# rensonnetg/microstructure_fingerprinting

Hardware: AMD Instinct MI355X
Metric: voxels/sec, 2-fascicle exhaustive NNLS, 782-atom x 200-measurement dictionary (higher is better)
Workload: dtype f64 (pairs ranked on split-f16 MFMA, short list re-evaluated in f64); 1 GPU; C2: 100000 voxels/GPU, 2 fascicles, 782 atoms x 200 measurements; voxels_per_gpu=100000, global_voxels=100000, atoms=782, measurements=200, ranks_in_group=1

## Files before the change

### microstructure_fingerprinting_amd/_lib.py

```python
import ctypes as C
import os

import numpy as np

_HERE = os.path.dirname(os.path.abspath(__file__))
LIB_PATH = os.path.join(_HERE, "libmfx.so")

MFX_OK, MFX_ERR_ARG, MFX_ERR_G_RANGE, MFX_ERR_NO_DEVICE, MFX_ERR_HIP, MFX_ERR_UNSUPPORTED, MFX_ERR_DIR_NORM = range(7)

_lib = None

EXPORTS = [
    "mfx_last_error", "mfx_device_count", "mfx_abi_version",
    "mfx_tables_create", "mfx_tables_destroy", "mfx_tables_num_atoms",
    "mfx_plan_create_multishell", "mfx_plan_create_explicit", "mfx_plan_destroy", "mfx_plan_status",
    "mfx_rotate", "mfx_rotate_dev", "mfx_rotate_cols", "mfx_rotate_cols_dev", "mfx_fit_batch", "mfx_fit_batch_rows", "mfx_fit_batch_volume", "mfx_volume_rows", "mfx_thread_release", "mfx_fit_batch_dev",
    "mfx_solve_exhaustive", "mfx_monte_carlo_average", "mfx_monte_carlo_average_dev", "mfx_cleanup_2fascicles", "mfx_cleanup_2fascicles_dev", "mfx_last_kernel_ms", "mfx_set_profiling", "mfx_debug_set_stamps", "mfx_debug_last_fallback_count", "mfx_debug_last_guard_count", "mfx_debug_last_counter", "mfx_debug_set_k2_screen", "mfx_debug_set_k2_wide", "mfx_debug_set_k2x_screen", "mfx_debug_set_k2_maxc", "mfx_debug_set_k2x_maxc", "mfx_debug_set_k2s_cap", "mfx_debug_set_k2s_images", "mfx_debug_set_k3_cap", "mfx_debug_set_force_generic", "mfx_debug_set_k3_screen",
]

MCF_EXPORTS = ["mfx_mcf_abi_version", "mfx_mcf_pgse", "mfx_mcf_dde"]

ROT2D_EXPORTS = ["mfx_rot2d_abi_version", "mfx_rot2d_create", "mfx_rot2d_destroy", "mfx_rot2d_rotate",
                 "mfx_rot2d_rotate_dev", "mfx_rot2d_rotate_cols", "mfx_rot2d_rotate_cols_dev"]

FIT2D_EXPORTS = ["mfx_fit2d_abi_version", "mfx_fit2d_max_atoms", "mfx_fit2d_batch_dev", "mfx_fit2d_batch",
                 "mfx_fit2d_debug_set_force_explicit"]

WFIT_EXPORTS = ["mfx_wfit_abi_version", "mfx_wfit_max_atoms", "mfx_wfit_batch_dev", "mfx_wfit_batch",
                "mfx_wfit_debug_set_force_explicit"]

PREDICT_EXPORTS = ["mfx_predict_abi_version", "mfx_predict_dev", "mfx_predict", "mfx_sos_noise_dev", "mfx_sos_noise"]

PROFILE_EXPORTS = ["mfx_profile_abi_version", "mfx_profile_cut", "mfx_profile_max_atoms", "mfx_profile_dev", "mfx_profile",
                   "mfx_pair_objectives_dev", "mfx_pair_objectives", "mfx_profile_debug_last_config"]

POST_EXPORTS = ["mfx_post_abi_version", "mfx_post_max_atoms", "mfx_post_dev", "mfx_post", "mfx_post_debug_last_config"]

WSOFT_EXPORTS = ["mfx_wsoft_abi_version", "mfx_wsoft_max_atoms", "mfx_wpost_dev", "mfx_wpost", "mfx_wprofile_dev", "mfx_wprofile",
                 "mfx_wpair_objectives_dev", "mfx_wpair_objectives"]

SOFT2D_EXPORTS = ["mfx_soft2d_abi_version", "mfx_soft2d_max_atoms", "mfx_post2d_dev", "mfx_post2d", "mfx_profile2d_dev",
# ... 80 lines not shown
    L.mfx_debug_last_guard_count.restype = C.c_int
    L.mfx_debug_last_counter.argtypes = [C.c_int]
    L.mfx_debug_last_counter.restype = C.c_int
    L.mfx_debug_set_k2x_maxc.argtypes = [C.c_int]
    L.mfx_debug_set_k2x_maxc.restype = None
    L.mfx_debug_set_k2_screen.argtypes = [C.c_int]
    L.mfx_debug_set_k2_screen.restype = None
    L.mfx_debug_set_k2_wide.argtypes = [C.c_int]
    L.mfx_debug_set_k2_wide.restype = None
    L.mfx_debug_set_k2x_screen.argtypes = [C.c_int]
    L.mfx_debug_set_k2x_screen.restype = None
    L.mfx_debug_set_k2_maxc.argtypes = [C.c_int]
    L.mfx_debug_set_k2_maxc.restype = None
    L.mfx_debug_set_k2s_cap.argtypes = [C.c_int]
    L.mfx_debug_set_k2s_cap.restype = None
    L.mfx_debug_set_k3_cap.argtypes = [C.c_int]
    L.mfx_debug_set_k3_cap.restype = None
    L.mfx_debug_set_force_generic.argtypes = [C.c_int]
    L.mfx_debug_set_force_generic.restype = None
    L.mfx_debug_set_k3_screen.argtypes = [C.c_int]
    L.mfx_debug_set_k3_screen.restype = None
    L.mfx_debug_set_k2s_images.argtypes = [C.c_int]
    L.mfx_debug_set_k2s_images.restype = None
    L.mfx_mcf_abi_version.restype = C.c_int
    for fn in ("mfx_mcf_pgse", "mfx_mcf_dde"):
        getattr(L, fn).argtypes = [dp, dp, C.c_int, dp, C.c_int64, dp, dp, C.c_int64, dp, C.c_double, dp]
        getattr(L, fn).restype = C.c_int
    L.mfx_rot2d_abi_version.restype = C.c_int
    L.mfx_rot2d_create.argtypes = [dp, C.c_int, ip, ip, C.c_int, ip, dp, ip, ip, ip, dp, C.c_int, ip, dp, dp, C.c_int,
                                   C.c_int, C.c_double, C.c_double, C.c_int, C.POINTER(vp)]
    L.mfx_rot2d_destroy.argtypes = [vp]
    L.mfx_rot2d_destroy.restype = None
    L.mfx_rot2d_rotate.argtypes = [vp, dp, C.c_int64, dp, ip]
    L.mfx_rot2d_rotate_dev.argtypes = [vp, vp, C.c_int64, vp, vp, vp]
    L.mfx_rot2d_rotate_cols.argtypes = [vp, dp, ip, C.c_int64, dp, ip]
    L.mfx_rot2d_rotate_cols_dev.argtypes = [vp, vp, vp, C.c_int64, vp, vp, vp]
    L.mfx_fit2d_abi_version.restype = C.c_int
    L.mfx_fit2d_max_atoms.argtypes = [vp, C.c_int]
    L.mfx_fit2d_batch_dev.argtypes = [vp, vp, vp, C.c_int, C.c_int64, vp, vp, vp]
    L.mfx_fit2d_batch.argtypes = [vp, dp, ip, bp, dp, C.c_int, C.c_int, dp, C.c_int64, dp, ip]
    L.mfx_fit2d_debug_set_force_explicit.argtypes = [C.c_int]
    L.mfx_fit2d_debug_set_force_explicit.restype = None
    L.mfx_wfit_abi_version.restype = C.c_int
    L.mfx_wfit_max_atoms.argtypes = [vp, C.c_int]
    L.mfx_wfit_batch_dev.argtypes = [vp, vp, vp, C.c_int64, vp, C.c_int, C.c_int64, vp, vp, vp]
    L.mfx_wfit_batch.argtypes = [vp, dp, dp, C.c_int64, ip, bp, dp, C.c_int, C.c_int, dp, C.c_int64, dp, ip]
# ... 156 lines not shown
```

### microstructure_fingerprinting_amd/csrc/fit_k2s.hip

```cpp
#pragma once
#include "fit_k2.hip"

typedef _Float16 h8 __attribute__((ext_vector_type(8)));
typedef _Float16 h4 __attribute__((ext_vector_type(4)));
typedef float f32x16 __attribute__((ext_vector_type(16)));
typedef float f32x2 __attribute__((ext_vector_type(2)));
typedef float f32x4 __attribute__((ext_vector_type(4)));
typedef int i32x4 __attribute__((ext_vector_type(4)));

#ifndef MFX_S_DC
#define MFX_S_DC 1.5e-5
#endif
template <int KS>
__host__ __device__ constexpr double mfx_s_dc() { return KS <= 13 ? (double)MFX_S_DC : 1.05 * (2.38e-6 + 3.0 * KS * 3.046e-7); }
#define MFX_S_DENMIN 1e-3
#define MFX_S_BOUND 0x40000000
#define MFX_S_GUARD 0.25

__device__ __forceinline__ unsigned long long mfx_nonneg_bits(double x) {
  return (unsigned long long)__double_as_longlong(x > 0.0 ? x : 0.0);
}

template <int CTRL>
__device__ __forceinline__ float mfx_dpp_max_f32(float v) {
// ... 12 lines not shown
  return (double)fmaxf(fmaxf(r0, r1), fmaxf(r2, r3));
}
__device__ __forceinline__ double mfx_rcp_nr(double x) {
  const double r0 = (double)__builtin_amdgcn_rcpf((float)x);
  return fma(r0, fma(-x, r0, 1.0), r0);
}

__device__ __forceinline__ double mfx_readlane_f64(double v, int l) {
  const long long b = __double_as_longlong(v);
  const unsigned lo = (unsigned)__builtin_amdgcn_readlane((int)(b & 0xffffffffll), l);
  const unsigned hi = (unsigned)__builtin_amdgcn_readlane((int)(b >> 32), l);
  return __longlong_as_double((long long)(((unsigned long long)hi << 32) | lo));
}

__device__ __forceinline__ void mfx_split16(float f, _Float16& hi, _Float16& lo) {
  asm("" : "+v"(f));
  const float h = __uint_as_float(__float_as_uint(f) & 0xffffe000u);
  hi = (_Float16)h;
  lo = (_Float16)(f - h);
}

#include "k2s_shared.h"
#include "k2s_tail16_map.h"

template <int KS, bool BR = false, int NB = 3, bool XC = false>
__global__ __launch_bounds__(512, 2) void mfx_fit_k2s_kernel(FitK2Args a) {
  constexpr int WG = 512, NW = 8;
  constexpr int MP = KS * 16;
  extern __shared__ double smem[];
  int tid = threadIdx.x;
  const int lane = tid & 63, wave = tid >> 6;
  const int lr = lane & 31, lh = lane >> 5;
  [[maybe_unused]] const int M = a.P.M;
  const int N = a.T.N, ldn = a.T.ldn;
  const int NP = (N + 31) & ~31;
  const int ntiles = NP >> 5;
  const int vox = a.vox_list ? a.vox_list[a.vox_base + blockIdx.x] : a.vox_base + (int)blockIdx.x;

  const K2sLds<KS, NB, BR, XC, NW * 64> L(smem, NP);
  K2S_UNPACK(L);
  const bool fused = !XC && (ntiles > 1) && (ntiles % NW == 1);
  const K2sVoxel VX = k2s_prologue<KS, NB, BR, XC, NW * 64, WG, !XC>(a, L, vox, tid, fused);
  const double y_sq = VX.y_sq, yx = VX.yx, ramp = VX.ramp, dc_eff = VX.dc_eff, mrg = VX.mrg, etol = VX.etol;
  (void)y_sq; (void)yx;
  const float2* __restrict__ tab32 = a.P.tab32s;
  auto tab32_at = [&](int ro, int n) -> float2 { return *(const float2*)((const char*)tab32 + ((unsigned)(ro + n) << 3)); };
  auto tab32x2_at = [&](int ro, int n) -> f32x4 { return *(const f32x4*)((const char*)tab32 + ((unsigned)(ro + n) << 3)); };
  auto push = [&](double S, int i, int j) { k2s_push(L, a.scap, S, i, j); };
// ... 35 lines not shown
```

### microstructure_fingerprinting_amd/csrc/k2s_launch.h

```cpp
#pragma once
#include "mfx_host.h"
#include "fit_k2s.hip"

template <int KS, bool BR, int NB>
static int launch_k2s_t(const FitK2Args& a, int nvox, hipStream_t st) {
  MfxThread& T = mfx_thread();
  const size_t lds = mfx_k2s_lds_bytes(KS, a.T.N, BR, NB);
  auto kern = mfx_fit_k2s_kernel<KS, BR, NB>;
  HIPCHK(hipFuncSetAttribute((const void*)kern, hipFuncAttributeMaxDynamicSharedMemorySize, (int)lds));
  StreamMem fbm(st);
  HIPCHK(fbm.alloc(sizeof(int) * ((size_t)nvox + 8)));
  int* fb = fbm.as<int>();
  HIPCHK(hipMemsetAsync(fb, 0, 8 * sizeof(int), st));
  if (int rc = mfx_prof_begin(st)) return rc;
  FitK2Args aa = a;
  aa.stamps = T.stamps;
  aa.fb_count = fb;
  aa.fb_list = fb + 8;
  aa.audit = fb + 2;
  aa.scap = T.k2s_cap ? T.k2s_cap : MFX_S_CAP;
  hipLaunchKernelGGL(kern, dim3(nvox), dim3(512), lds, st, aa);
  HIPCHK(hipGetLastError());
  if (int rc = mfx_prof_end(st)) return rc;
  FitK2Args ab = a;
  ab.vox_list = fb + 8;
  ab.list_count = fb;
  if (int rc = mfx_launch_k2_f64(ab, nvox, st, false)) return rc;
  if (int rc = mfx_fb_accumulate(fb, 2, st)) return rc;
  return mfx_fb_accumulate_audit(fb + 2, st);
}

#define MFX_K2S_TU(KS_, NAME_)                                                            \
  int NAME_(const FitK2Args& a, int nvox, hipStream_t st, bool br, int NB) {              \
    if (NB == 3) return br ? launch_k2s_t<KS_, true, 3>(a, nvox, st) : launch_k2s_t<KS_, false, 3>(a, nvox, st); \
    return br ? launch_k2s_t<KS_, true, 2>(a, nvox, st) : launch_k2s_t<KS_, false, 2>(a, nvox, st);              \
  }
```

### microstructure_fingerprinting_amd/csrc/k2s_round.h

```cpp
    const bool tail = K2S_ROUND_MODE == 0 ? (ntiles - round * NW == 1) && (ntiles > 1) : K2S_ROUND_MODE == 1;
    const int rt = tail ? round * NW : round * NW + wave;
    const bool rt_valid = rt < ntiles;
    const int rtc = rt_valid ? rt : 0;
    h8 afh[KS], afl[KS];
#if K2S_ROUND_MODE == 1
    const bool t16 = N - 32 * (ntiles - 1) <= 16;
    if (!t16)
#endif
    {
      const int n = rtc * 32 + lr;
      const int nn = min(n, ldn - 1);
      double a2 = 0.0, ay = 0.0;
      float um1 = 0.0f;
      if constexpr (XC) um1 = (rt_valid && n < N) ? -s_uf[n] : 0.0f;
      mfx_static_for<0, KS>([&](auto kc) {
        constexpr int ks = decltype(kc)::value;
        float2 d[8];
#pragma unroll
        for (int j = 0; j < 8; ++j) d[j] = tab32_at(s_rs[16 * ks + 8 * lh + j], nn);
        h8 vh, vl;
#pragma unroll
        for (int j = 0; j < 8; ++j) {
          float fv = fmaf(d[j].y, s_t0f[16 * ks + 8 * lh + j], d[j].x);
          fv = rt_valid ? fv : 0.0f;
// ... 21 lines not shown
      const double z = ay * inv;
      if (rt_valid && lh == 0) {
        s_Zf[n] = act ? (float)z : -1e30f;
        s_cs[n] = (act && a2 > 0.0) ? (float)nrm : 0.0f;
      }
      double sb = (act && z > 0.0) ? z * z : 0.0;
#pragma unroll
      for (int o = 16; o > 0; o >>= 1) sb = fmax(sb, __shfl_xor(sb, o));
      sb = mfx_readlane_f64(sb, 0);
      if (lane == 0 && sb - mrg > 0.0) atomicMax(&s_thr[0], mfx_nonneg_bits(sb - mrg));
      }
    }

    double thr = 0.0, thr_rows = -1.0;
#ifdef MFX_STAMPS_RND
    int dbg_flagged = 0, dbg_groups = 0;
#endif
    const float DCF = XC ? (float)((mfx_s_dc<KS>() + 2e-6) * ramp) * (1.0f + 2e-7f)
                         : (float)mfx_s_dc<KS>() + 2e-6f;
    auto pq_of = [&](float z, float rth, float& P, float& Q) {
      P = fminf(1.0f, fmaxf(z, 0.0f) * rth);
      Q = __builtin_amdgcn_sqrtf(fmaxf(0.0f, fmaf(-P, P, 1.0f) - 1.2e-7f)) * (1.0f - 3e-7f);
    };
    unsigned long long sc_thr = 0ull;
    float sc_z2 = 0.0f, sc_s = 0.0f;
    auto scan_pre = [&](int ct) {
      const int j = ct * 32 + lr;
      sc_thr = s_thr[0];
      sc_z2 = s_Zf[NP + j];
      sc_s = s_cs[NP + j];
    };
#ifdef MFX_STAMPS_SCAN
    int dbg_calls = 0;
#define MFX_SCAN_T(k) do { if (a.stamps && round == 0 && dbg_calls == 1 && wave == 0 && lane == 0) a.stamps[(size_t)blockIdx.x * 16 + (k)] = __builtin_amdgcn_s_memtime(); } while (0)
#else
#define MFX_SCAN_T(k) do { } while (0)
#endif
    auto scan_pair = [&](const int i, const int j, const float accv, const double z2, const double n2d) {
      const double n12 = (double)s_cs[i] * n2d;
      const double c = n12 > 0.0 ? (double)accv * mfx_rcp_nr(n12) : 0.0;
      const double z1 = (double)s_Zf[i];
      const double e1 = fma(-c, z2, z1);
      const double e2 = fma(-c, z1, z2);
      const double den = fma(-c, c, 1.0);
      const double num = fma(z2, e2, z1 * e1);
      const bool pos = (e1 > -etol) & (e2 > -etol);
      const bool wellc = (den >= MFX_S_DENMIN) & (c >= 0.0);
      const bool hit = pos & wellc & (fma(-thr, den, num) >= 0.0);
      const bool near = pos & !wellc;
      if (!__any(hit | near)) return;
      double S = -1.0;
      if (hit) {
        S = num * mfx_rcp_nr(den);
      } else if (near) {
        const double dlo = den - 2.0 * dc_eff - dc_eff * dc_eff;
        const double u1 = fabs(e1) + etol, u2 = fabs(e2) + etol;
        S = (dlo > 0.0 && c > -0.5) ? fmin(fma(z2, z2, u1 * u1 / dlo), fma(z1, z1, u2 * u2 / dlo)) + mrg : 1e300;
      }
      bool feas = hit;
      double q1x = 0.0, q2x = 0.0;
      if constexpr (XC) {
        q1x = (double)s_uf[i] * mfx_rcp_nr(fmax((double)s_cs[i], 1e-300));
        q2x = (double)s_uf[NP + j] * mfx_rcp_nr(fmax(n2d, 1e-300));
// ... 18 lines not shown
            else if (f1 < -etol || f2 < -etol) slist = -1.0;
          }
        }
      }
      const double smax = mfx_wave_max_down(fmax(sraise, 0.0));
      if (smax - 2.0 * mrg > thr) {
        thr = smax - 2.0 * mrg;
        if (lane == 0) atomicMax(&s_thr[0], mfx_nonneg_bits(thr));
      }
      if ((hit | near) && slist >= thr) push(slist, i, hit ? j : (j | MFX_S_BOUND));
#ifdef MFX_STAMPS_SCAN
      if (a.stamps && round == 0 && dbg_calls == 1 && wave == 0 && lane == 0) {
        unsigned long long* st = a.stamps + (size_t)blockIdx.x * 16;
        if (st[15] < 8) st[4 + st[15]] = __builtin_amdgcn_s_memtime();
        ++st[15];
      }
#endif
    };
    auto scan_main = [&](const f32x16& acc, int ct) {
#ifdef MFX_STAMPS_SCAN
      ++dbg_calls;
#endif
      MFX_SCAN_T(0);
      {
        if (((rt << 8) | ct) == aud_key) {
          const unsigned h = k2s_audit_hash(vox);
          const int ga = (h >> 16) & 15;
          float v = acc[0];
#pragma unroll
          for (int g = 1; g < 16; ++g) v = (ga == g) ? acc[g] : v;
          if (lane == (int)((h >> 20) & 63)) ((float*)(s_red + 30))[0] = v;
        }
      }
      const int j = ct * 32 + lr;
      thr = fmax(thr, __longlong_as_double((long long)sc_thr));
      const float rth = __builtin_amdgcn_rsqf(fmaxf((float)thr * (1.0f - 2e-7f), 1e-30f)) * (1.0f + 4e-7f);
      float* pqw = s_pq + wave * 64;
      if (thr > thr_rows) {
        thr_rows = thr;
        if (lane < 32) {
          const float z1 = s_Zf[rtc * 32 + lane], n1 = s_cs[rtc * 32 + lane];
          float P, Q;
          pq_of(z1, rth, P, Q);
          const bool ok = n1 > 0.0f;
          pqw[lane] = ok ? (P + DCF) * n1 : 0.0f;
          pqw[32 + lane] = ok ? Q * ((1.0f - DCF) * n1) : 1e18f;
// ... 18 lines not shown
      if (__any(fmaxf(fmaxf(mm[0], mm[1]), fmaxf(mm[2], mm[3])) >= 0.0f)) {
        MFX_SCAN_T(2);
#ifdef MFX_STAMPS_RND
        ++dbg_flagged;
#endif
        const double z2 = (double)s_Zf[NP + j], n2d = (double)s_cs[NP + j];
#pragma unroll 1
        for (int q = 0; q < 4; ++q) {
          if (!__any(mm[q] >= 0.0f)) continue;
          const f32x4 p1q = *(const f32x4*)(pqw + 8 * q + 4 * lh);
          const f32x4 q1q = *(const f32x4*)(pqw + 32 + 8 * q + 4 * lh);
#pragma unroll 1
          for (int gg = 0; gg < 4; ++gg) {
            const int g = 4 * q + gg;
            if (!__any(fmaf(-q1q[gg], q2, fmaf(p1q[gg], p2, -acc[g])) >= 0.0f)) continue;
#ifdef MFX_STAMPS_RND
            ++dbg_groups;
#endif
            scan_pair(rt * 32 + (g & 3) + 8 * (g >> 2) + 4 * lh, j, acc[g], z2, n2d);
          }
        }
        MFX_SCAN_T(3);
      }
    };
    auto scan_tile = [&](const f32x16& acc, int ct) { scan_pre(ct); scan_main(acc, ct); };

#ifdef MFX_EXP_NOTAIL
    if (tail) continue;
#endif
    if (tail) {
#if K2S_ROUND_MODE == 1
      if (!t16)
#endif
      {
#ifdef MFX_STAMPS_RND
      if (a.stamps && tid == 0 && round < 4) a.stamps[(size_t)blockIdx.x * 16 + 2 * round + 1] = __builtin_amdgcn_s_memtime();
#endif
      thr = __longlong_as_double((long long)s_thr[0]);
      }
      [[maybe_unused]] double* const s_bs2 = s_red + 8 + wave;
      [[maybe_unused]] int* const s_bn2 = (int*)(s_red + 16) + 8 + wave;
      if constexpr (!XC) { if (lane == 0) { *s_bs2 = 0.0; *s_bn2 = 0; } }
#if K2S_ROUND_MODE == 1
      if (t16) {
        constexpr int NS16 = k2s_t16_steps(KS);
        const int g16 = lane >> 4;
        h8 a16h[NS16], a16l[NS16];
        {
// ... 278 lines not shown
    const int gq = KS * grp + (tg >> 4);
    const bool gact = (tg >> 4) < KS;
    auto gen_load = [&](int ch) {
      const int nn = min(ch * 32 + 2 * (tg & 15), ldn - 2);
      const int q = gact ? gq : KS * grp;
#pragma unroll
      for (int e = 0; e < 8; ++e) gd[e] = tab32x2_at(s_rs[MP + 8 * q + e], nn);
    };
#ifndef MFX_XC_GT
#define MFX_XC_GT 0
#endif
    constexpr bool GT = KS <= 13 && (!XC || MFX_XC_GT);
    float g_t[GT ? 8 : 1];
    if constexpr (GT) {
#pragma unroll
      for (int e = 0; e < 8; ++e) g_t[e] = s_t0f[MP + 8 * (gact ? gq : KS * grp) + e];
    }
    auto gen_store = [&](int ch, int buf) {
      if (gact) {
        const int c0 = 2 * (tg & 15);
        h8 hi0, lo0, hi1, lo1;
        float gu0 = 0.0f, gu1 = 0.0f;
        if constexpr (XC) { gu0 = s_uf[NP + ch * 32 + c0]; gu1 = s_uf[NP + ch * 32 + c0 + 1]; }
#pragma unroll
        for (int e = 0; e < 8; ++e) {
          const float t = GT ? g_t[GT ? e : 0] : s_t0f[MP + 8 * gq + e];
          _Float16 x, y;
          float v0 = fmaf(gd[e][1], t, gd[e][0]), v1 = fmaf(gd[e][3], t, gd[e][2]);
          if constexpr (XC) { if (e == 7) { const bool spare = (gq == 2 * KS - 1); v0 = spare ? gu0 : v0; v1 = spare ? gu1 : v1; } }
          mfx_split16(v0, x, y);
          hi0[e] = x; lo0[e] = y;
          mfx_split16(v1, x, y);
          hi1[e] = x; lo1[e] = y;
        }
        const int off = (gq * 32 + c0) << 3;
        _Float16* dh = sBh + buf * KS * 512 + off;
        _Float16* dl = sBl + buf * KS * 512 + off;
        *(h8*)dh = hi0; *(h8*)(dh + 8) = hi1;
        *(h8*)dl = lo0; *(h8*)(dl + 8) = lo1;
      }
    };
    f32x16 acc;
#pragma unroll
    for (int g = 0; g < 16; ++g) acc[g] = 0.0f;
    auto mfma_chunk = [&](int buf) {
#pragma unroll
      for (int g = 0; g < 16; ++g) acc[g] = 0.0f;
      const _Float16* bhp = sBh + buf * KS * 512 + lane * 8;
      const _Float16* blp = sBl + buf * KS * 512 + lane * 8;
      h8 bh = *(const h8*)bhp, bl = *(const h8*)blp;
      mfx_static_for<0, KS>([&](auto kc) {
        constexpr int ks = decltype(kc)::value;
        h8 bhn = bh, bln = bl;
        if constexpr (ks + 1 < KS) {
          bhn = *(const h8*)(bhp + (ks + 1) * 512);
          bln = *(const h8*)(blp + (ks + 1) * 512);
        }
        acc = __builtin_amdgcn_mfma_f32_32x32x16_f16(afh[ks], bh, acc, 0, 0, 0);
        acc = __builtin_amdgcn_mfma_f32_32x32x16_f16(afh[ks], bl, acc, 0, 0, 0);
        acc = __builtin_amdgcn_mfma_f32_32x32x16_f16(afl[ks], bh, acc, 0, 0, 0);
        bh = bhn; bl = bln;
        __builtin_amdgcn_sched_barrier(0);
      });
    };

    if (round == 0) MFX_STAMP(3);
#ifdef MFX_STAMPS_RND
    if (a.stamps && tid == 0 && round < 4) a.stamps[(size_t)blockIdx.x * 16 + 2 * round + 1] = __builtin_amdgcn_s_memtime();
#endif
    if constexpr (NB == 3) {
      gen_load(0);
      gen_store(0, 0);
      if (grp == 0) {
        if (ntiles > 1) { gen_load(1); gen_store(1, 1); }
        if (ntiles > 2) gen_load(2);
      } else if (ntiles > 1) {
        gen_load(1);
      }
      __syncthreads();
      if (round == 0) MFX_STAMP(4);
      thr = __longlong_as_double((long long)s_thr[0]);
      int b0 = 0;
#ifdef MFX_EXP_NOGEN
      const bool exp_gen = round == 0;
#else
      constexpr bool exp_gen = true;
#endif
      for (int c = 0; c <= ntiles; ++c) {
#ifdef MFX_STAMPS_HS
#ifndef MFX_HS_ROUND
#define MFX_HS_ROUND 1
#define MFX_HS_C0 10
#endif
        if (a.stamps && round == MFX_HS_ROUND && c >= MFX_HS_C0 && c < MFX_HS_C0 + 16 && tid == 0) a.stamps[(size_t)blockIdx.x * 16 + c - MFX_HS_C0] = __builtin_amdgcn_s_memtime();
#endif
        const int b1 = b0 == 2 ? 0 : b0 + 1, b2 = b1 == 2 ? 0 : b1 + 1;
        if (grp == 0) {
          if (c < ntiles) {
            if (rt_valid) { mfma_chunk(b0); scan_pre(c); }
            if (exp_gen && c + 2 < ntiles) gen_store(c + 2, b2);
            if (rt_valid) scan_main(acc, c);
            if (exp_gen && c + 3 < ntiles) gen_load(c + 3);
          }
        } else {
          if (c >= 1 && rt_valid) scan_pre(c - 1);
          if (exp_gen && c + 1 < ntiles) gen_store(c + 1, b1);
          if (c >= 1 && rt_valid) scan_main(acc, c - 1);
          if (exp_gen && c + 2 < ntiles) gen_load(c + 2);
          if (c < ntiles && rt_valid) mfma_chunk(b0);
        }
        asm volatile("s_waitcnt lgkmcnt(0)\n\ts_barrier" ::: "memory");
        b0 = b1;
      }
    } else {
      gen_load(0);
      gen_store(0, 0);
      if (grp == 1 && ntiles > 1) { gen_load(1); gen_store(1, 1); }
      __syncthreads();
      if (round == 0) MFX_STAMP(4);
      thr = __longlong_as_double((long long)s_thr[0]);
      for (int hs = 0; hs <= 2 * ntiles; ++hs) {
        if ((hs & 1) == grp) {
          const int c = (hs - grp) >> 1;
          if (c < ntiles) {
            if (c + 1 + grp < ntiles) gen_load(c + 1 + grp);
            if (rt_valid) mfma_chunk(c & 1);
          }
        } else {
          const int c = (hs - 1 - grp) >> 1;
          if (c >= 0 && c < ntiles) {
            if (c + 1 + grp < ntiles) gen_store(c + 1 + grp, (c + 1 + grp) & 1);
// ... 12 lines not shown
```

### microstructure_fingerprinting_amd/csrc/mfx_api.hip

```cpp
#include "mfx_host.h"

#include <algorithm>
#include <chrono>
#include <cmath>
#include <cstdarg>
#include <cstdio>
#include <cstdlib>
#include <cstring>
#include <memory>
#include <string>
#include <vector>

#include "fit_small.hip"
#include "extras.hip"
#include "rotate.hip"
#include "solve_generic.hip"
#include "solve_k3.hip"
#include "fit_k3.hip"
#include "mc_average.hip"
#include "cleanup.hip"
#include "mfx_device.h"

MfxThread& mfx_thread() {
  static thread_local MfxThread t;
// ... 189 lines not shown
}
extern "C" void mfx_set_profiling(int enabled) { mfx_thread().profiling = enabled != 0; }
extern "C" double mfx_last_kernel_ms(void) {
  MfxThread& T = mfx_thread();
  if (!T.ev_valid || !T.ev0 || !T.ev1 || T.ev_launches == 0) return -1.0;
  if (hipEventSynchronize(T.ev1) != hipSuccess) return -1.0;
  float ms = 0;
  if (hipEventElapsedTime(&ms, T.ev0, T.ev1) != hipSuccess) return -1.0;
  return (double)ms / T.ev_launches;
}
extern "C" int mfx_debug_last_fallback_count(void) { return fb_read(0); }
extern "C" int mfx_debug_last_guard_count(void) { return fb_read(1); }
extern "C" int mfx_debug_last_counter(int which) { return (which >= 0 && which < MFX_NCOUNTERS) ? fb_read(which) : -1; }
extern "C" void mfx_debug_set_k2_screen(int enabled) { mfx_thread().k2_screen = enabled ? 1 : 0; }
extern "C" void mfx_debug_set_k2_wide(int mode) { mfx_thread().k2_wide = mode == 1 ? 1 : (mode == 0 ? 0 : 2); }
extern "C" void mfx_debug_set_k2x_screen(int on) { mfx_thread().k2x_screen = on ? 1 : 0; }
extern "C" void mfx_debug_set_stamps(void* dev_ptr) { mfx_thread().stamps = (unsigned long long*)dev_ptr; }
extern "C" void mfx_debug_set_k2_maxc(int maxc) { mfx_thread().k2_maxc = (maxc < 0 || maxc > MFX_MAXC) ? MFX_MAXC : maxc; }
extern "C" void mfx_debug_set_k2x_maxc(int maxc) { mfx_thread().k2x_maxc = (maxc < 0 || maxc > MFX_XMAXC) ? MFX_XMAXC : maxc; }
extern "C" void mfx_debug_set_k3_cap(int cap) { mfx_thread().k3_cap = cap > 0 ? cap : 0; }
extern "C" void mfx_debug_set_force_generic(int enabled) { mfx_thread().force_generic = enabled ? 1 : 0; }
extern "C" void mfx_debug_set_k3_screen(int enabled) { mfx_thread().k3_screen = enabled ? 1 : 0; }
extern "C" void mfx_debug_set_k2s_images(int nb) { mfx_thread().k2s_nb = (nb == 2) ? 2 : 0; }
extern "C" void mfx_debug_set_k2s_cap(int cap) {
  int c = 4;
  while (2 * c <= cap) c *= 2;
  mfx_thread().k2s_cap = (cap <= 0 || c >= MFX_S_CAP) ? 0 : c;
}

struct mfx_tables {
  int device = 0;
  TablesDev d{};
  std::vector<double> h_x, h_G, h_Y;
  double scr_scale = 1.0;
  std::vector<int> h_off;
  void* dx = nullptr;
  void* doff = nullptr;
  void* dtab = nullptr;
  void* dtab32 = nullptr;
  void* dG = nullptr;
  ~mfx_tables() {
    (void)hipFree(dx); (void)hipFree(doff); (void)hipFree(dtab); (void)hipFree(dtab32); (void)hipFree(dG);
  }
};

struct mfx_plan {
// ... 277 lines not shown
  const size_t MP = (size_t)KS * 16, NP = ((size_t)N + 31) / 32 * 32;
  return mfx_k2w_lds_bytes(KS, N, bracket, NB, TL) + 4 * MP + 8 * NP;
}

static int launch_k2(const FitK2Args& a, int nvox, hipStream_t st) {
  MfxThread& T = mfx_thread();
  if (T.k2_screen < 0) { const char* e = getenv("MFX_K2_SCREEN"); T.k2_screen = (e && e[0] == '0') ? 0 : 1; }
  if (T.k2_wide < 0) { const char* e = getenv("MFX_K2_WIDE"); T.k2_wide = e ? (e[0] == '1' ? 1 : (e[0] == '0' ? 0 : 2)) : 2; }
  const int M = a.P.M;
  const bool br = a.P.any_bracket != 0;
  if (T.k2_screen && mfx_k2_f64_fits(a)) {
    const bool wide_ok = T.k2_wide != 0;
    if (M > 256 && M <= 560 && wide_ok) {
      if (M <= 384 && mfx_k2w_lds_bytes(24, a.T.N, br, 1, 1) <= 160 * 1024) return mfx_launch_k2w_ks24(a, nvox, st, br);
      if (mfx_k2w_lds_bytes(35, a.T.N, br, 1, 1) <= 160 * 1024) return mfx_launch_k2w_ks35(a, nvox, st, br);
    }
    if (M <= 256) {
      if (T.k2_wide == 1 && M > 128) {
        if (M <= 208 && mfx_k2w_lds_bytes(13, a.T.N, br, 2, 2) <= 160 * 1024) return mfx_launch_k2w_ks13(a, nvox, st, br);
        if (mfx_k2w_lds_bytes(16, a.T.N, br, 2, 2) <= 160 * 1024) return mfx_launch_k2w_ks16(a, nvox, st, br);
      }
      const int KSm = M <= 64 ? 4 : (M <= 128 ? 8 : (M <= 208 ? 13 : 16));
      const int NB = (T.k2s_nb != 2 && mfx_k2s_lds_bytes(KSm, a.T.N, br, 3) <= 160 * 1024) ? 3 : (mfx_k2s_lds_bytes(KSm, a.T.N, br, 2) <= 160 * 1024 ? 2 : 0);
      if (NB) {
        if (KSm == 4) return mfx_launch_k2s_ks4(a, nvox, st, br, NB);
        if (KSm == 8) return mfx_launch_k2s_ks8(a, nvox, st, br, NB);
        if (KSm == 13) return mfx_launch_k2s_ks13(a, nvox, st, br, NB);
        return mfx_launch_k2s_ks16(a, nvox, st, br, NB);
      }
    }
  }
  if (int rc = mfx_launch_k2_f64(a, nvox, st, true)) return rc;
  return MFX_OK;
}

struct ExtrasHost {
  ExtrasDev d{};
  void* dx = nullptr;
  void* dG = nullptr;
  hipStream_t st = nullptr;
  ExtrasHost() = default;
  ExtrasHost(const ExtrasHost&) = delete;
  ExtrasHost& operator=(const ExtrasHost&) = delete;
  int build(int M, int has_csf, int E, const double* d_sig_csf, const double* d_sig_ear, hipStream_t stream) {
    const int NX = has_csf + E;
    st = stream;
    d.NX = NX; d.has_csf = has_csf; d.E = E; d.x = nullptr; d.Gxx = nullptr;
    if (NX == 0) return MFX_OK;
    if (has_csf && !d_sig_csf) return fail(MFX_ERR_ARG, "sig_csf missing");
    if (E && !d_sig_ear) return fail(MFX_ERR_ARG, "sig_ear missing");
    HIPCHK(mfx_scratch_alloc(&dx, sizeof(double) * (size_t)M * NX, st));
// ... 1071 lines not shown
```

### microstructure_fingerprinting_amd/csrc/mfx_host.h

```cpp
#pragma once
#include "../../include/mfx.h"

#include <hip/hip_runtime.h>

#include <string>
#include <vector>

#include "class_batch.h"
#include "fit_k2.hip"
#include "fit_k2x.hip"

#define MFX_NCOUNTERS 12

struct MfxThread {
  std::string err;
  hipEvent_t ev0 = nullptr, ev1 = nullptr;
  int ev_launches = 0;
  bool ev_valid = false;
  bool profiling = false;
  unsigned long long* stamps = nullptr;
  int k2_pipe = -1;
  int k2_maxc = MFX_MAXC;
  int k2x_maxc = MFX_XMAXC;
  int k2s_nb = 0;
  int k2s_cap = 0;
  int force_generic = 0;
  int k3_screen = 1;
  int k3_cap = 0;
  int k3_batch = -1;
  int k2_screen = -1;
  int k2x_screen = -1;
  int k2_wide = -1;
  int* fb_dev = nullptr;
  int* fb_host = nullptr;
  int fb_device = -1;
  hipEvent_t fb_event = nullptr;
  bool fb_pending = false;
  void* stage[2] = {nullptr, nullptr};
  size_t stage_bytes = 0;
  hipStream_t s_copy = nullptr, s_comp = nullptr;
  hipEvent_t ev_h2d[2] = {nullptr, nullptr};
  int pipe_device = -1;
  void* pool[6] = {nullptr, nullptr, nullptr, nullptr, nullptr, nullptr};
  size_t pool_bytes[6] = {0, 0, 0, 0, 0, 0};
  struct Arena {
    int device = -1;
    hipStream_t stream = nullptr;
    std::vector<void*> blocks;
// ... 130 lines not shown
template <class Steps>
int mfx_rob_iterate(const Steps& s, int n_iter, const MfxRobHostCount* host) {
  if (int rc = s.first_fit()) return rc;
  s.step_done();
  for (int it = 0; it < n_iter; ++it) {
    if (int rc = s.reweight(it)) return rc;
    s.step_done();
    if (host) {
      int32_t nc = 0;
      HIPCHK(hipMemcpy(&nc, host->d_nchanged + it, sizeof(int32_t), hipMemcpyDeviceToHost));
      host->n_changed[it] += nc;
      *host->n_iter_used = std::max<int32_t>(*host->n_iter_used, it + 1);
      if (nc == 0 && (it > 0 || host->has_w0)) break;
    }
    if (int rc = s.refit()) return rc;
    s.step_done();
  }
  return MFX_OK;
}

int mfx_launch_k2_f64(const FitK2Args& a, int nvox, hipStream_t st, bool record_events);
bool mfx_k2_f64_fits(const FitK2Args& a);
size_t mfx_k2s_lds_bytes(int KS, int N, bool bracket, int NB);
int mfx_launch_k2s_ks4(const FitK2Args& a, int nvox, hipStream_t st, bool br, int NB);
int mfx_launch_k2s_ks8(const FitK2Args& a, int nvox, hipStream_t st, bool br, int NB);
int mfx_launch_k2s_ks13(const FitK2Args& a, int nvox, hipStream_t st, bool br, int NB);
int mfx_launch_k2s_ks16(const FitK2Args& a, int nvox, hipStream_t st, bool br, int NB);
size_t mfx_k2sx_lds_bytes(int KS, int N, bool bracket, int NB);
int mfx_launch_k2sx_ks8(const FitK2Args& a, int nvox, hipStream_t st, bool br);
int mfx_launch_k2sx_ks13(const FitK2Args& a, int nvox, hipStream_t st, bool br);
size_t mfx_k2w_lds_bytes(int KS, int N, bool bracket, int NB, int TL);
size_t mfx_k2wx_lds_bytes(int KS, int N, bool bracket, int NB, int TL);
int mfx_launch_k2wx_ks24(const FitK2Args& a, int nvox, hipStream_t st, bool br);
int mfx_launch_k2wx_ks35(const FitK2Args& a, int nvox, hipStream_t st, bool br);
int mfx_launch_k2w_ks13(const FitK2Args& a, int nvox, hipStream_t st, bool br);
int mfx_launch_k2w_ks16(const FitK2Args& a, int nvox, hipStream_t st, bool br);
int mfx_launch_k2w_ks24(const FitK2Args& a, int nvox, hipStream_t st, bool br);
int mfx_launch_k2w_ks35(const FitK2Args& a, int nvox, hipStream_t st, bool br);
int mfx_launch_k2x(const FitK2XArgs& a, int nvox, hipStream_t st);
```

Before: 1.198 million voxels/s.

## Fold per-pair screening bound into spare MFMA K-slots of the split-f16 GEMM

Uses the padding columns of the K dimension (when 16*KS exceeds M by two or more) to carry per-row and per-column bound constants (p, q), so the MFMA accumulator directly yields a sign-testable screening value. The scan no longer loads per-column z/norm values for every tile. A cheap integer min-over-sign test decides whether any pair needs examination, and only flagged groups rebuild the exact f64 correlation. This adds per-tile row-constant refreshes when the threshold rises, extra LDS (s_pq), and rounding-guard logic whose conservativeness must hold for correctness.

```diff
diff --git a/include/mfx_k2s_debug.h b/include/mfx_k2s_debug.h
--- /dev/null
+++ b/include/mfx_k2s_debug.h
@@ -0,0 +1,12 @@
+#ifndef MFX_K2S_DEBUG_H
+#define MFX_K2S_DEBUG_H
+#ifdef __cplusplus
+extern "C" {
+#endif
+
+void mfx_debug_set_k2s_fold(int on);
+
+#ifdef __cplusplus
+}
+#endif
+#endif
diff --git a/microstructure_fingerprinting_amd/_lib.py b/microstructure_fingerprinting_amd/_lib.py
--- a/microstructure_fingerprinting_amd/_lib.py
+++ b/microstructure_fingerprinting_amd/_lib.py
@@ -17,6 +17,8 @@
     "mfx_rotate", "mfx_rotate_dev", "mfx_rotate_cols", "mfx_rotate_cols_dev", "mfx_fit_batch", "mfx_fit_batch_rows", "mfx_fit_batch_volume", "mfx_volume_rows", "mfx_thread_release", "mfx_fit_batch_dev",
     "mfx_solve_exhaustive", "mfx_monte_carlo_average", "mfx_monte_carlo_average_dev", "mfx_cleanup_2fascicles", "mfx_cleanup_2fascicles_dev", "mfx_last_kernel_ms", "mfx_set_profiling", "mfx_debug_set_stamps", "mfx_debug_last_fallback_count", "mfx_debug_last_guard_count", "mfx_debug_last_counter", "mfx_debug_set_k2_screen", "mfx_debug_set_k2_wide", "mfx_debug_set_k2x_screen", "mfx_debug_set_k2_maxc", "mfx_debug_set_k2x_maxc", "mfx_debug_set_k2s_cap", "mfx_debug_set_k2s_images", "mfx_debug_set_k3_cap", "mfx_debug_set_force_generic", "mfx_debug_set_k3_screen",
 ]
+
+K2S_DEBUG_EXPORTS = ["mfx_debug_set_k2s_fold"]
 
 MCF_EXPORTS = ["mfx_mcf_abi_version", "mfx_mcf_pgse", "mfx_mcf_dde"]
 
@@ -143,6 +145,8 @@
     L.mfx_debug_set_k3_screen.restype = None
     L.mfx_debug_set_k2s_images.argtypes = [C.c_int]
     L.mfx_debug_set_k2s_images.restype = None
+    L.mfx_debug_set_k2s_fold.argtypes = [C.c_int]
+    L.mfx_debug_set_k2s_fold.restype = None
     L.mfx_mcf_abi_version.restype = C.c_int
     for fn in ("mfx_mcf_pgse", "mfx_mcf_dde"):
         getattr(L, fn).argtypes = [dp, dp, C.c_int, dp, C.c_int64, dp, dp, C.c_int64, dp, C.c_double, dp]
diff --git a/microstructure_fingerprinting_amd/csrc/fit_k2s.hip b/microstructure_fingerprinting_amd/csrc/fit_k2s.hip
--- a/microstructure_fingerprinting_amd/csrc/fit_k2s.hip
+++ b/microstructure_fingerprinting_amd/csrc/fit_k2s.hip
@@ -58,8 +58,9 @@
 
 #include "k2s_shared.h"
 #include "k2s_tail16_map.h"
+#include "k2s_fold.h"
 
-template <int KS, bool BR = false, int NB = 3, bool XC = false>
+template <int KS, bool BR = false, int NB = 3, bool XC = false, bool FOLD = false>
 __global__ __launch_bounds__(512, 2) void mfx_fit_k2s_kernel(FitK2Args a) {
   constexpr int WG = 512, NW = 8;
   constexpr int MP = KS * 16;
diff --git a/microstructure_fingerprinting_amd/csrc/k2s_fold.h b/microstructure_fingerprinting_amd/csrc/k2s_fold.h
--- /dev/null
+++ b/microstructure_fingerprinting_amd/csrc/k2s_fold.h
@@ -0,0 +1,57 @@
+#pragma once
+
+#if defined(__HIPCC__) || defined(__CUDACC__)
+#define K2S_FOLD_HD __host__ __device__ inline
+#else
+#define K2S_FOLD_HD inline
+#endif
+
+#define K2S_FOLD_LOLO 9.5367431640625e-7f
+#define K2S_FOLD_PIPE 9.2e-7f
+
+struct K2sFoldPQ { float p, q; };
+
+K2S_FOLD_HD unsigned k2s_fold_bits(float f) { return __builtin_bit_cast(unsigned, f); }
+K2S_FOLD_HD float k2s_fold_float(unsigned u) { return __builtin_bit_cast(float, u); }
+
+K2S_FOLD_HD float k2s_fold_dcf(float dcf) { return dcf + K2S_FOLD_LOLO * ((1.0f + dcf) * (1.0f + dcf)) + K2S_FOLD_PIPE; }
+
+K2S_FOLD_HD float k2s_fold_up(float f) {
+  const float a = __builtin_ceilf(f * 16777216.0f) * 5.9604644775390625e-8f;
+  const float b = k2s_fold_float((k2s_fold_bits(f) + 3u) & ~3u);
+  return f < 0.125f ? a : b;
+}
+K2S_FOLD_HD float k2s_fold_down(float f) {
+  const float a = __builtin_floorf(f * 16777216.0f) * 5.9604644775390625e-8f;
+  const float b = k2s_fold_float(k2s_fold_bits(f) & ~3u);
+  return f < 0.125f ? a : b;
+}
+K2S_FOLD_HD float k2s_fold_hi(float f) { return k2s_fold_float(k2s_fold_bits(f) & 0xffffe000u); }
+K2S_FOLD_HD float k2s_fold_lo(float f) { return f - k2s_fold_hi(f); }
+
+K2S_FOLD_HD float k2s_fold_sqrt(float x) {
+#if defined(__HIP_DEVICE_COMPILE__)
+  return __builtin_amdgcn_sqrtf(x);
+#else
+  return __builtin_sqrtf(x);
+#endif
+}
+
+K2S_FOLD_HD K2sFoldPQ k2s_fold_consts(float z, float n, float rth, float dcf) {
+  const float P = __builtin_fminf(1.0f, __builtin_fmaxf(z, 0.0f) * rth);
+  const float Q = k2s_fold_sqrt(__builtin_fmaxf(0.0f, __builtin_fmaf(-P, P, 1.0f) - 1.2e-7f)) * (1.0f - 3e-7f);
+  K2sFoldPQ c;
+  c.p = k2s_fold_up((P + dcf) * n);
+  c.q = k2s_fold_down(Q * ((1.0f - dcf) * n));
+  c.p = n < 1.0f ? k2s_fold_up(3.0f * n) : c.p;
+  c.q = n < 1.0f ? -k2s_fold_up(n + n) : c.q;
+  c.p = n > 0.0f ? c.p : -1.0f;
+  c.q = n > 0.0f ? c.q : 256.0f;
+  return c;
+}
+
+K2S_FOLD_HD double k2s_fold_pure(float accp, float p1, float q1, float p2, float q2) {
+  const double pp = (double)p1 * (double)p2 - (double)k2s_fold_lo(p1) * (double)k2s_fold_lo(p2);
+  const double qq = (double)q1 * (double)q2 - (double)k2s_fold_lo(q1) * (double)k2s_fold_lo(q2);
+  return ((double)accp + pp) - qq;
+}
diff --git a/microstructure_fingerprinting_amd/csrc/k2s_launch.h b/microstructure_fingerprinting_amd/csrc/k2s_launch.h
--- a/microstructure_fingerprinting_amd/csrc/k2s_launch.h
+++ b/microstructure_fingerprinting_amd/csrc/k2s_launch.h
@@ -2,11 +2,11 @@
 #include "mfx_host.h"
 #include "fit_k2s.hip"
 
-template <int KS, bool BR, int NB>
+template <int KS, bool BR, int NB, bool FOLD = false>
 static int launch_k2s_t(const FitK2Args& a, int nvox, hipStream_t st) {
   MfxThread& T = mfx_thread();
   const size_t lds = mfx_k2s_lds_bytes(KS, a.T.N, BR, NB);
-  auto kern = mfx_fit_k2s_kernel<KS, BR, NB>;
+  auto kern = mfx_fit_k2s_kernel<KS, BR, NB, false, FOLD>;
   HIPCHK(hipFuncSetAttribute((const void*)kern, hipFuncAttributeMaxDynamicSharedMemorySize, (int)lds));
   StreamMem fbm(st);
   HIPCHK(fbm.alloc(sizeof(int) * ((size_t)nvox + 8)));
@@ -31,7 +31,10 @@
 }
 
 #define MFX_K2S_TU(KS_, NAME_)                                                            \
-  int NAME_(const FitK2Args& a, int nvox, hipStream_t st, bool br, int NB) {              \
+  int NAME_(const FitK2Args& a, int nvox, hipStream_t st, bool br, int NB, bool fold) {   \
+    if constexpr (KS_ <= 13) {                                                            \
+      if (NB == 3 && fold) return br ? launch_k2s_t<KS_, true, 3, true>(a, nvox, st) : launch_k2s_t<KS_, false, 3, true>(a, nvox, st); \
+    }                                                                                     \
     if (NB == 3) return br ? launch_k2s_t<KS_, true, 3>(a, nvox, st) : launch_k2s_t<KS_, false, 3>(a, nvox, st); \
     return br ? launch_k2s_t<KS_, true, 2>(a, nvox, st) : launch_k2s_t<KS_, false, 2>(a, nvox, st);              \
   }
diff --git a/microstructure_fingerprinting_amd/csrc/k2s_round.h b/microstructure_fingerprinting_amd/csrc/k2s_round.h
--- a/microstructure_fingerprinting_amd/csrc/k2s_round.h
+++ b/microstructure_fingerprinting_amd/csrc/k2s_round.h
@@ -67,13 +67,46 @@
       P = fminf(1.0f, fmaxf(z, 0.0f) * rth);
       Q = __builtin_amdgcn_sqrtf(fmaxf(0.0f, fmaf(-P, P, 1.0f) - 1.2e-7f)) * (1.0f - 3e-7f);
     };
+#if K2S_ROUND_MODE == 2
+    constexpr bool FD = FOLD && !XC && NB == 3 && KS <= 13;
+#else
+    constexpr bool FD = false;
+#endif
+    [[maybe_unused]] const float DCFF = k2s_fold_dcf(DCF);
+    [[maybe_unused]] unsigned kbh = 0u, kbl = 0u;
+    [[maybe_unused]] double fold_accd = 0.0;
     unsigned long long sc_thr = 0ull;
     float sc_z2 = 0.0f, sc_s = 0.0f;
     auto scan_pre = [&](int ct) {
       const int j = ct * 32 + lr;
       sc_thr = s_thr[0];
-      sc_z2 = s_Zf[NP + j];
-      sc_s = s_cs[NP + j];
+      if constexpr (!FD) {
+        sc_z2 = s_Zf[NP + j];
+        sc_s = s_cs[NP + j];
+      }
+    };
+    [[maybe_unused]] auto fold_rows = [&]() {
+      thr = fmax(thr, __longlong_as_double((long long)sc_thr));
+      if (thr > thr_rows) {
+        thr_rows = thr;
+        const float rth = __builtin_amdgcn_rsqf(fmaxf((float)thr * (1.0f - 2e-7f), 1e-30f)) * (1.0f + 4e-7f);
+        const K2sFoldPQ c = k2s_fold_consts(s_Zf[rtc * 32 + lr], s_cs[rtc * 32 + lr], rth, DCFF);
+        float* pqw = s_pq + wave * 64;
+        if (lh == 0) { pqw[lr] = c.p; pqw[32 + lr] = c.q; }
+        _Float16 ph, pl, qh, ql;
+        mfx_split16(-c.p, ph, pl);
+        mfx_split16(c.q, qh, ql);
+        h8 vh = afh[KS - 1], vl = afl[KS - 1];
+        vh[6] = lh ? ph : vh[6]; vh[7] = lh ? qh : vh[7];
+        vl[6] = lh ? pl : vl[6]; vl[7] = lh ? ql : vl[7];
+        afh[KS - 1] = vh; afl[KS - 1] = vl;
+      }
+    };
+    [[maybe_unused]] auto fold_col = [&](float& p2, float& q2) {
+      typedef _Float16 h2 __attribute__((ext_vector_type(2)));
+      const h2 ch = __builtin_bit_cast(h2, __shfl(kbh, lr + 32)), cl = __builtin_bit_cast(h2, __shfl(kbl, lr + 32));
+      p2 = (float)ch[0] + (float)cl[0];
+      q2 = (float)ch[1] + (float)cl[1];
     };
 #ifdef MFX_STAMPS_SCAN
     int dbg_calls = 0;
@@ -83,7 +116,9 @@
 #endif
     auto scan_pair = [&](const int i, const int j, const float accv, const double z2, const double n2d) {
       const double n12 = (double)s_cs[i] * n2d;
-      const double c = n12 > 0.0 ? (double)accv * mfx_rcp_nr(n12) : 0.0;
+      double accd = (double)accv;
+      if constexpr (FD) accd = fold_accd;
+      const double c = n12 > 0.0 ? accd * mfx_rcp_nr(n12) : 0.0;
       const double z1 = (double)s_Zf[i];
       const double e1 = fma(-c, z2, z1);
       const double e2 = fma(-c, z1, z2);
@@ -148,6 +183,57 @@
       ++dbg_calls;
 #endif
       MFX_SCAN_T(0);
+      if constexpr (FD) {
+        const int j = ct * 32 + lr;
+        const float* pqw = s_pq + wave * 64;
+        if (((rt << 8) | ct) == aud_key) {
+          const unsigned h = k2s_audit_hash(vox);
+          const int ga = (h >> 16) & 15;
+          float v = acc[0];
+#pragma unroll
+          for (int g = 1; g < 16; ++g) v = (ga == g) ? acc[g] : v;
+          const int il = (ga & 3) + 8 * (ga >> 2) + 4 * lh;
+          float p2, q2;
+          fold_col(p2, q2);
+          const double vd = k2s_fold_pure(v, pqw[il], pqw[32 + il], p2, q2);
+          if (lane == (int)((h >> 20) & 63)) ((float*)(s_red + 30))[0] = (float)vd;
+        }
+        int mi[4];
+#pragma unroll
+        for (int q = 0; q < 4; ++q)
+          mi[q] = min(min(__float_as_int(acc[4 * q]), __float_as_int(acc[4 * q + 1])), min(__float_as_int(acc[4 * q + 2]), __float_as_int(acc[4 * q + 3])));
+        MFX_SCAN_T(1);
+        if (__any(min(min(mi[0], mi[1]), min(mi[2], mi[3])) <= 0)) {
+          MFX_SCAN_T(2);
+#ifdef MFX_STAMPS_RND
+          ++dbg_flagged;
+#endif
+          thr = fmax(thr, __longlong_as_double((long long)s_thr[0]));
+          const float rth = __builtin_amdgcn_rsqf(fmaxf((float)thr * (1.0f - 2e-7f), 1e-30f)) * (1.0f + 4e-7f);
+          const float z2f = s_Zf[NP + j], n2 = s_cs[NP + j];
+          const K2sFoldPQ f2 = k2s_fold_consts(z2f, n2, rth, DCFF);
+          float p2, q2;
+          fold_col(p2, q2);
+          const float dp = f2.p - p2, dq = f2.q - q2;
+          const double z2 = (double)z2f, n2d = (double)n2;
+#pragma unroll 1
+          for (int q = 0; q < 4; ++q) {
+            const f32x4 p1q = *(const f32x4*)(pqw + 8 * q + 4 * lh);
+            const f32x4 q1q = *(const f32x4*)(pqw + 32 + 8 * q + 4 * lh);
+#pragma unroll 1
+            for (int gg = 0; gg < 4; ++gg) {
+              const int g = 4 * q + gg;
+              if (!__any(fmaf(-q1q[gg], dq, fmaf(p1q[gg], dp, -acc[g])) >= 0.0f)) continue;
+#ifdef MFX_STAMPS_RND
+              ++dbg_groups;
+#endif
+              fold_accd = k2s_fold_pure(acc[g], p1q[gg], q1q[gg], p2, q2);
+              scan_pair(rt * 32 + (g & 3) + 8 * (g >> 2) + 4 * lh, j, acc[g], z2, n2d);
+            }
+          }
+          MFX_SCAN_T(3);
+        }
+      } else {
       {
         if (((rt << 8) | ct) == aud_key) {
           const unsigned h = k2s_audit_hash(vox);
@@ -212,8 +298,9 @@
         }
         MFX_SCAN_T(3);
       }
-    };
-    auto scan_tile = [&](const f32x16& acc, int ct) { scan_pre(ct); scan_main(acc, ct); };
+      }
+    };
+    auto scan_tile =[&](const f32x16& acc, int ct) { scan_pre(ct); scan_main(acc, ct); };
 
 #ifdef MFX_EXP_NOTAIL
     if (tail) continue;
@@ -538,12 +625,36 @@
         h8 hi0, lo0, hi1, lo1;
         float gu0 = 0.0f, gu1 = 0.0f;
         if constexpr (XC) { gu0 = s_uf[NP + ch * 32 + c0]; gu1 = s_uf[NP + ch * 32 + c0 + 1]; }
+        [[maybe_unused]] unsigned long long f_thr = 0ull;
+        [[maybe_unused]] float2 f_z = {0.0f, 0.0f}, f_n = {0.0f, 0.0f};
+        [[maybe_unused]] K2sFoldPQ f_c0 = {0.0f, 0.0f}, f_c1 = {0.0f, 0.0f};
+        if constexpr (FD) {
+          if (gq == 2 * KS - 1) {
+            f_thr = s_thr[0];
+            f_z = *(const float2*)(s_Zf + NP + ch * 32 + c0);
+            f_n = *(const float2*)(s_cs + NP + ch * 32 + c0);
+          }
+        }
 #pragma unroll
         for (int e = 0; e < 8; ++e) {
           const float t = GT ? g_t[GT ? e : 0] : s_t0f[MP + 8 * gq + e];
           _Float16 x, y;
           float v0 = fmaf(gd[e][1], t, gd[e][0]), v1 = fmaf(gd[e][3], t, gd[e][2]);
           if constexpr (XC) { if (e == 7) { const bool spare = (gq == 2 * KS - 1); v0 = spare ? gu0 : v0; v1 = spare ? gu1 : v1; } }
+          if constexpr (FD) {
+            if (e == 6) {
+              if (gq == 2 * KS - 1) {
+                const float rth = __builtin_amdgcn_rsqf(fmaxf((float)__longlong_as_double((long long)f_thr) * (1.0f - 2e-7f), 1e-30f)) * (1.0f + 4e-7f);
+                f_c0 = k2s_fold_consts(f_z.x, f_n.x, rth, DCFF);
+                f_c1 = k2s_fold_consts(f_z.y, f_n.y, rth, DCFF);
+              }
+            }
+            if (e >= 6) {
+              const bool spare = (gq == 2 * KS - 1);
+              v0 = spare ? (e == 6 ? f_c0.p : f_c0.q) : v0;
+              v1 = spare ? (e == 6 ? f_c1.p : f_c1.q) : v1;
+            }
+          }
           mfx_split16(v0, x, y);
           hi0[e] = x; lo0[e] = y;
           mfx_split16(v1, x, y);
@@ -572,9 +683,18 @@
           bhn = *(const h8*)(bhp + (ks + 1) * 512);
           bln = *(const h8*)(blp + (ks + 1) * 512);
         }
+        if constexpr (FD && ks == KS - 1) {
+          acc = __builtin_amdgcn_mfma_f32_32x32x16_f16(afh[ks], bl, acc, 0, 0, 0);
+          acc = __builtin_amdgcn_mfma_f32_32x32x16_f16(afl[ks], bh, acc, 0, 0, 0);
+          acc = __builtin_amdgcn_mfma_f32_32x32x16_f16(afh[ks], bh, acc, 0, 0, 0);
+          typedef unsigned u32x4 __attribute__((ext_vector_type(4)));
+          kbh = __builtin_bit_cast(u32x4, bh)[3];
+          kbl = __builtin_bit_cast(u32x4, bl)[3];
+        } else {
         acc = __builtin_amdgcn_mfma_f32_32x32x16_f16(afh[ks], bh, acc, 0, 0, 0);
         acc = __builtin_amdgcn_mfma_f32_32x32x16_f16(afh[ks], bl, acc, 0, 0, 0);
         acc = __builtin_amdgcn_mfma_f32_32x32x16_f16(afl[ks], bh, acc, 0, 0, 0);
+        }
         bh = bhn; bl = bln;
         __builtin_amdgcn_sched_barrier(0);
       });
@@ -596,6 +716,7 @@
       __syncthreads();
       if (round == 0) MFX_STAMP(4);
       thr = __longlong_as_double((long long)s_thr[0]);
+      if constexpr (FD) sc_thr = (unsigned long long)__double_as_longlong(thr);
       int b0 = 0;
 #ifdef MFX_EXP_NOGEN
       const bool exp_gen = round == 0;
@@ -613,16 +734,19 @@
         const int b1 = b0 == 2 ? 0 : b0 + 1, b2 = b1 == 2 ? 0 : b1 + 1;
         if (grp == 0) {
           if (c < ntiles) {
-            if (rt_valid) { mfma_chunk(b0); scan_pre(c); }
+            if constexpr (FD) { if (rt_valid) fold_rows(); }
+            if (rt_valid) { mfma_chunk(b0); if constexpr (!FD) scan_pre(c); }
             if (exp_gen && c + 2 < ntiles) gen_store(c + 2, b2);
             if (rt_valid) scan_main(acc, c);
+            if constexpr (FD) { if (rt_valid) scan_pre(c); }
             if (exp_gen && c + 3 < ntiles) gen_load(c + 3);
           }
         } else {
-          if (c >= 1 && rt_valid) scan_pre(c - 1);
+          if ((FD || c >= 1) && rt_valid) scan_pre(c - 1);
           if (exp_gen && c + 1 < ntiles) gen_store(c + 1, b1);
           if (c >= 1 && rt_valid) scan_main(acc, c - 1);
           if (exp_gen && c + 2 < ntiles) gen_load(c + 2);
+          if constexpr (FD) { if (c < ntiles && rt_valid) fold_rows(); }
           if (c < ntiles && rt_valid) mfma_chunk(b0);
         }
         asm volatile("s_waitcnt lgkmcnt(0)\n\ts_barrier" ::: "memory");
diff --git a/microstructure_fingerprinting_amd/csrc/mfx_api.hip b/microstructure_fingerprinting_amd/csrc/mfx_api.hip
--- a/microstructure_fingerprinting_amd/csrc/mfx_api.hip
+++ b/microstructure_fingerprinting_amd/csrc/mfx_api.hip
@@ -1,4 +1,5 @@
 #include "mfx_host.h"
+#include "../../include/mfx_k2s_debug.h"
 
 #include <algorithm>
 #include <chrono>
@@ -235,6 +236,7 @@
 extern "C" void mfx_debug_set_force_generic(int enabled) { mfx_thread().force_generic = enabled ? 1 : 0; }
 extern "C" void mfx_debug_set_k3_screen(int enabled) { mfx_thread().k3_screen = enabled ? 1 : 0; }
 extern "C" void mfx_debug_set_k2s_images(int nb) { mfx_thread().k2s_nb = (nb == 2) ? 2 : 0; }
+extern "C" void mfx_debug_set_k2s_fold(int on) { mfx_thread().k2s_fold = on ? 1 : 0; }
 extern "C" void mfx_debug_set_k2s_cap(int cap) {
   int c = 4;
   while (2 * c <= cap) c *= 2;
@@ -558,11 +560,12 @@
       }
       const int KSm = M <= 64 ? 4 : (M <= 128 ? 8 : (M <= 208 ? 13 : 16));
       const int NB = (T.k2s_nb != 2 && mfx_k2s_lds_bytes(KSm, a.T.N, br, 3) <= 160 * 1024) ? 3 : (mfx_k2s_lds_bytes(KSm, a.T.N, br, 2) <= 160 * 1024 ? 2 : 0);
+      const bool fold = T.k2s_fold != 0 && 16 * KSm - M >= 2;
       if (NB) {
-        if (KSm == 4) return mfx_launch_k2s_ks4(a, nvox, st, br, NB);
-        if (KSm == 8) return mfx_launch_k2s_ks8(a, nvox, st, br, NB);
-        if (KSm == 13) return mfx_launch_k2s_ks13(a, nvox, st, br, NB);
-        return mfx_launch_k2s_ks16(a, nvox, st, br, NB);
+        if (KSm == 4) return mfx_launch_k2s_ks4(a, nvox, st, br, NB, fold);
+        if (KSm == 8) return mfx_launch_k2s_ks8(a, nvox, st, br, NB, fold);
+        if (KSm == 13) return mfx_launch_k2s_ks13(a, nvox, st, br, NB, fold);
+        return mfx_launch_k2s_ks16(a, nvox, st, br, NB, fold);
       }
     }
   }
diff --git a/microstructure_fingerprinting_amd/csrc/mfx_host.h b/microstructure_fingerprinting_amd/csrc/mfx_host.h
--- a/microstructure_fingerprinting_amd/csrc/mfx_host.h
+++ b/microstructure_fingerprinting_amd/csrc/mfx_host.h
@@ -24,6 +24,7 @@
   int k2x_maxc = MFX_XMAXC;
   int k2s_nb = 0;
   int k2s_cap = 0;
+  int k2s_fold = 1;
   int force_generic = 0;
   int k3_screen = 1;
   int k3_cap = 0;
@@ -200,10 +201,10 @@
 int mfx_launch_k2_f64(const FitK2Args& a, int nvox, hipStream_t st, bool record_events);
 bool mfx_k2_f64_fits(const FitK2Args& a);
 size_t mfx_k2s_lds_bytes(int KS, int N, bool bracket, int NB);
-int mfx_launch_k2s_ks4(const FitK2Args& a, int nvox, hipStream_t st, bool br, int NB);
-int mfx_launch_k2s_ks8(const FitK2Args& a, int nvox, hipStream_t st, bool br, int NB);
-int mfx_launch_k2s_ks13(const FitK2Args& a, int nvox, hipStream_t st, bool br, int NB);
-int mfx_launch_k2s_ks16(const FitK2Args& a, int nvox, hipStream_t st, bool br, int NB);
+int mfx_launch_k2s_ks4(const FitK2Args& a, int nvox, hipStream_t st, bool br, int NB, bool fold);
+int mfx_launch_k2s_ks8(const FitK2Args& a, int nvox, hipStream_t st, bool br, int NB, bool fold);
+int mfx_launch_k2s_ks13(const FitK2Args& a, int nvox, hipStream_t st, bool br, int NB, bool fold);
+int mfx_launch_k2s_ks16(const FitK2Args& a, int nvox, hipStream_t st, bool br, int NB, bool fold);
 size_t mfx_k2sx_lds_bytes(int KS, int N, bool bracket, int NB);
 int mfx_launch_k2sx_ks8(const FitK2Args& a, int nvox, hipStream_t st, bool br);
 int mfx_launch_k2sx_ks13(const FitK2Args& a, int nvox, hipStream_t st, bool br);
```

Measured after the change: 1.182 million voxels/s. 1.3% lower.
